# jolibrain/jolineedle

Measured on AMD Instinct MI355X. Metric: glimpse-patches/sec (448px, seq-len 20) REINFORCE step, higher is better.
Workload: dtype f32; 1 GPU; configs[2]/[3]: REINFORCE rollout, gpt-nano + yolox-nano encoder, 448px, seq-len 20, --enable-stop, 64 agents/GPU x 1 GPU, 4480x4480 synthetic images, forced non-STOP actions (S=T); global_batch=64, seq_len=20

## Files before the change

### include/jnroll.h

```cpp
#ifndef JNROLL_H
#define JNROLL_H

#include <stddef.h>
#include <stdint.h>

#ifdef __cplusplus
extern "C" {
#endif

#define JN_ABI_VERSION 2

enum {
  JN_OK = 0,
  JN_EINVAL = -1,
  JN_ENOMEM = -2,
  JN_EHIP = -3,
  JN_ENOTFOUND = -4,
  JN_ESTATE = -5
};

enum { JN_MODE_GREEDY = 0, JN_MODE_SAMPLE = 1, JN_MODE_FORCED = 2 };

enum { JN_NET_GPT_BACKBONE = 0, JN_NET_DETECTOR = 1 };

// ... 193 lines not shown

int jn_gpt_forward(jn_ctx* ctx, const float* patches_dev, const int64_t* actions_dev, const int64_t* classes_dev,
                   const int64_t* positions_dev, const float* prev_emb_dev, int B, int T, int Tp,
                   float* logits_dev, float* final_emb_dev, void* stream);
int jn_detect(jn_ctx* ctx, const float* patches_dev, int N, float* boxes_dev,
              int32_t* counts_dev, float* raw_dev, void* stream);
int jn_set_det_candidates(jn_ctx* ctx, int all);

int jn_detector_step(jn_ctx* ctx, const float* patches_dev, int N, const float* targets_dev, int nb,
                     float loss_scale, float* metrics_dev, void* stream);
#define JN_DETLOSS_MAX_BOXES 1024
int jn_set_det_loss_boxes(jn_ctx* ctx, int all);
int jn_detector_forward(jn_ctx* ctx, const float* patches_dev, int N, const float* targets_dev, int nb, int pass,
                        int n_pass, float* metrics_dev, float* boxes_dev, int32_t* counts_dev, float* fpn0_dev,
                        float* fpn1_dev, float* fpn2_dev, void* stream);
int jn_detector_backward(jn_ctx* ctx, int pass, const float* dloss_dev, float scale, void* stream);
int jn_detector_eval_loss(jn_ctx* ctx, const float* patches_dev, int N, const float* targets_dev, int nb,
                          float* metrics_dev, float* boxes_dev, int32_t* counts_dev, float* fpn0_dev, float* fpn1_dev,
                          float* fpn2_dev, void* stream);
int jn_optimizer_step_group(jn_ctx* ctx, int group, float lr, float weight_decay, float clip_value,
                            float grad_scale, void* stream);

int jn_rollout(jn_ctx* ctx, int mode, const int64_t* forced_actions_dev,
               const int64_t* start_positions_dev, uint64_t seed, int do_detection,
               int stop_early, const jn_rollout_out* out, void* stream);
int jn_set_rollout_positions(jn_ctx* ctx, int by_token);
int jn_teacher_actions(const int64_t* positions_dev, const uint8_t* visited_dev, const uint8_t* targets_dev, int B, int Gh,
                       int Gw, uint8_t* sets_dev, void* stream);
int jn_teacher_walks(const int64_t* bboxes_dev, const int64_t* start_positions_dev, int B, int nb, int Gh, int Gw, int P,
                     int T, int min_keypoints, int max_keypoints, int binomial_keypoints, uint64_t seed, int capacity,
                     int64_t* positions_dev, int64_t* current_actions_dev, int64_t* next_actions_dev, int64_t* labels_dev,
                     float* masks_dev, float* local_bboxes_dev, int32_t* n_steps_dev, uint8_t* targets_dev,
                     int64_t* cells_dev, float* bboxes_yolox_dev, int32_t* offsets_dev, void* stream);
int jn_set_rollout_teacher(jn_ctx* ctx, const uint8_t* targets_dev, uint8_t* sets_dev);
int jn_rollout_steps(jn_ctx* ctx, int* n_steps, void* stream);

int jn_last_timing(jn_ctx* ctx, int what, float* ms);
int jn_set_profiling(jn_ctx* ctx, int enabled);

#ifdef __cplusplus
}
#endif
#endif
```

### jolineedle_amd/_lib.py

```python
import ctypes as C
import os
from pathlib import Path

_LIB = None
LIB_PATH = Path(__file__).resolve().parent / "lib" / "libjnroll.so"

JN_MODE_GREEDY, JN_MODE_SAMPLE, JN_MODE_FORCED = 0, 1, 2
JN_NET_GPT_BACKBONE, JN_NET_DETECTOR = 0, 1


class LibraryNotBuilt(RuntimeError):
    pass


class JnError(RuntimeError):
    pass


class JnConfig(C.Structure):
    _fields_ = [("struct_size", C.c_int32), ("device", C.c_int32),
                ("n_layer", C.c_int32), ("n_head", C.c_int32), ("n_embd", C.c_int32),
                ("block_size", C.c_int32), ("n_actions", C.c_int32), ("patch_size", C.c_int32),
                ("use_pos_emb", C.c_int32), ("no_patch_emb", C.c_int32), ("concat_emb", C.c_int32),
                ("decoder_pos_encoding", C.c_int32), ("pos_emb_size", C.c_int32),
# ... 84 lines not shown
    "jn_pool_walk_detections": (C.c_int, [C.c_void_p] * 6 + [C.c_int] * 9 + [C.c_void_p] * 5),
    "jn_detection_cells": (C.c_int, [C.c_void_p, C.c_void_p] + [C.c_int] * 6 + [C.c_uint64, C.c_int] + [C.c_void_p] * 5),
    "jn_gather_patches_views": (C.c_int, [C.c_void_p, C.c_int, C.c_void_p, C.c_void_p, C.c_void_p, C.c_int, C.c_int, C.c_int,
                                          C.c_int, C.c_int, C.c_void_p]),
    "jn_backbone_forward": (C.c_int, [C.c_void_p, C.c_int, C.c_void_p, C.c_int, C.c_int, C.c_void_p, C.c_void_p,
                                      C.c_void_p, C.c_void_p]),
    "jn_read_tensor": (C.c_int, [C.c_void_p, C.c_char_p, C.c_void_p, C.c_size_t]),
    "jn_embed_patches": (C.c_int, [C.c_void_p, C.c_void_p, C.c_int, C.c_void_p, C.c_void_p]),
    "jn_reinforce_step": (C.c_int, [C.c_void_p, C.c_int, C.c_void_p, C.c_void_p, C.c_uint64, C.c_int,
                                    C.POINTER(JnTrainOpts), C.POINTER(JnRolloutOut), C.c_void_p, C.c_void_p]),
    "jn_supervised_step": (C.c_int, [C.c_void_p, C.c_void_p, C.c_void_p, C.c_void_p, C.c_void_p, C.c_void_p, C.c_void_p,
                                     C.c_int, C.c_int, C.c_float, C.c_void_p, C.c_void_p, C.c_void_p]),
    "jn_supervised_forward": (C.c_int, [C.c_void_p, C.c_void_p, C.c_void_p, C.c_void_p, C.c_void_p, C.c_int, C.c_int,
                                        C.c_void_p, C.c_void_p, C.c_void_p]),
    "jn_supervised_backward": (C.c_int, [C.c_void_p, C.c_void_p, C.c_void_p]),
    "jn_optimizer_step": (C.c_int, [C.c_void_p, C.c_float, C.c_float, C.c_float, C.c_float, C.c_void_p]),
    "jn_arena_info": (C.c_int, [C.c_void_p, C.POINTER(C.c_size_t), C.POINTER(C.c_size_t)]),
    "jn_set_grad_arena": (C.c_int, [C.c_void_p, C.c_void_p, C.c_size_t]),
    "jn_read_param": (C.c_int, [C.c_void_p, C.c_char_p, C.c_void_p, C.c_size_t]),
    "jn_zero_grad": (C.c_int, [C.c_void_p, C.c_void_p]),
    "jn_backbone_backward": (C.c_int, [C.c_void_p, C.c_int, C.c_void_p, C.c_int, C.c_void_p, C.c_void_p, C.c_void_p,
                                       C.c_void_p]),
    "jn_read_grad": (C.c_int, [C.c_void_p, C.c_char_p, C.c_void_p, C.c_size_t]),
    "jn_gpt_forward": (C.c_int, [C.c_void_p, C.c_void_p, C.c_void_p, C.c_void_p, C.c_void_p, C.c_void_p, C.c_int, C.c_int,
                                 C.c_int, C.c_void_p, C.c_void_p, C.c_void_p]),
    "jn_detect": (C.c_int, [C.c_void_p, C.c_void_p, C.c_int, C.c_void_p, C.c_void_p, C.c_void_p, C.c_void_p]),
    "jn_set_det_candidates": (C.c_int, [C.c_void_p, C.c_int]),
    "jn_set_det_loss_boxes": (C.c_int, [C.c_void_p, C.c_int]),
    "jn_rollout": (C.c_int, [C.c_void_p, C.c_int, C.c_void_p, C.c_void_p, C.c_uint64, C.c_int, C.c_int,
                             C.POINTER(JnRolloutOut), C.c_void_p]),
    "jn_set_rollout_positions": (C.c_int, [C.c_void_p, C.c_int]),
    "jn_teacher_actions": (C.c_int, [C.c_void_p, C.c_void_p, C.c_void_p, C.c_int, C.c_int, C.c_int, C.c_void_p, C.c_void_p]),
    "jn_teacher_walks": (C.c_int, [C.c_void_p, C.c_void_p] + [C.c_int] * 9 + [C.c_uint64, C.c_int] + [C.c_void_p] * 12),
    "jn_set_rollout_teacher":(C.c_int, [C.c_void_p, C.c_void_p, C.c_void_p]),
    "jn_rollout_steps": (C.c_int, [C.c_void_p, C.POINTER(C.c_int), C.c_void_p]),
    "jn_last_timing": (C.c_int, [C.c_void_p, C.c_int, C.POINTER(C.c_float)]),
    "jn_set_profiling": (C.c_int, [C.c_void_p, C.c_int]),
    "jn_detector_step": (C.c_int, [C.c_void_p, C.c_void_p, C.c_int, C.c_void_p, C.c_int, C.c_float, C.c_void_p, C.c_void_p]),
    "jn_detector_forward": (C.c_int, [C.c_void_p, C.c_void_p, C.c_int, C.c_void_p, C.c_int, C.c_int, C.c_int, C.c_void_p,
                                      C.c_void_p, C.c_void_p, C.c_void_p, C.c_void_p, C.c_void_p, C.c_void_p]),
    "jn_detector_backward": (C.c_int, [C.c_void_p, C.c_int, C.c_void_p, C.c_float, C.c_void_p]),
    "jn_optimizer_step_group": (C.c_int, [C.c_void_p, C.c_int, C.c_float, C.c_float, C.c_float, C.c_float, C.c_void_p]),
    "jn_reinforce_forward": (C.c_int, [C.c_void_p, C.c_int, C.c_void_p, C.c_void_p, C.c_uint64, C.c_int,
                                       C.POINTER(JnRolloutOut), C.c_void_p]),
    "jn_reinforce_backward": (C.c_int, [C.c_void_p, C.c_void_p, C.c_void_p, C.c_void_p]),
    "jn_arena_segment": (C.c_int, [C.c_void_p, C.c_char_p, C.POINTER(C.c_size_t), C.POINTER(C.c_size_t)]),
    "jn_export_arena": (C.c_int, [C.c_void_p, C.c_int, C.c_void_p, C.c_size_t, C.c_int, C.c_void_p]),
    "jn_import_arena": (C.c_int, [C.c_void_p, C.c_int, C.c_void_p, C.c_size_t, C.c_void_p]),
    "jn_set_dropout": (C.c_int, [C.c_void_p, C.c_float, C.c_uint64]),
    "jn_set_freeze": (C.c_int, [C.c_void_p, C.c_int]),
    "jn_optimizer_steps": (C.c_int, [C.c_void_p, C.c_int, C.POINTER(C.c_int), C.c_int]),
    "jn_supervised_metrics": (C.c_int, [C.c_void_p, C.c_void_p, C.c_void_p, C.c_void_p, C.c_int, C.c_int, C.c_int, C.c_float, C.c_int,
                                        C.c_void_p, C.c_void_p, C.c_void_p, C.c_void_p]),
    "jn_supervised_eval": (C.c_int, [C.c_void_p] * 7 + [C.c_int, C.c_int, C.c_float, C.c_int] + [C.c_void_p] * 5),
    "jn_detector_eval_loss": (C.c_int, [C.c_void_p, C.c_void_p, C.c_int, C.c_void_p, C.c_int] + [C.c_void_p] * 7),
}


def load_library(path=None):
    global _LIB
    if _LIB is not None and path is None:
        return _LIB
    p = Path(path or os.environ.get("JNROLL_LIB", LIB_PATH))
    if not p.exists():
        raise LibraryNotBuilt(
            f"{p} not found: the HIP extension is not built. Run `bash jolineedle_amd/csrc/build.sh` "
# ... 26 lines not shown
```

### jolineedle_amd/csrc/api_net.hip

```cpp
#include <algorithm>
#include <cstring>

#include "jn_internal.h"

using namespace jnr;

extern "C"
__global__ void bn_eval_table_kernel(const float* __restrict__ gamma, const float* __restrict__ beta,
                                     const float* __restrict__ rmean, const float* __restrict__ rvar, ChanTab t0,
                                     ChanTab t1, int C, float eps) {
  const int c = blockIdx.x * blockDim.x + threadIdx.x;
  if (c >= C) return;
  const float sc = gamma[c] / sqrtf(rvar[c] + eps);
  const float sh = beta[c] - rmean[c] * sc;
  t0.sc[c] = sc; t0.sh[c] = sh; t0.fl[c] = 1.0f;
  if (t1.sc) { t1.sc[c] = sc; t1.sh[c] = sh; t1.fl[c] = 1.0f; }
}

extern "C"
__global__ void fill_kernel(float* p, float v, long long n) {
  const long long i = (long long)blockIdx.x * blockDim.x + threadIdx.x;
  if (i < n) p[i] = v;
}

// ... 469 lines not shown
      } else {
        if (!st.red_by)
          launch_bn_bwd_reduce(gp_out, gld_out, ptr(op.out), net.act_dtype, ld(op.out), tab(op.out), save + 2 * cw.stat_off, cw.cout,
                               M, red, rep_stride, s, sb);
        launch_bn_bwd_consts(red, rep_stride, (double)M, cw.gamma_dev, cw.beta_dev, save + 2 * cw.stat_off, consts,
                             grad_of(ctx, cw.gamma_dev), grad_of(ctx, cw.beta_dev), cw.cout, s, sb, st.red_by & 1);
      }
      float* gw = grad_of(ctx, cw.w_dev);
      if (st.route == BR_PW_FUSED || st.route == BR_PW_FUSED_HALVES) {
        const int parts = st.route == BR_PW_FUSED ? 1 : 2, pc = cw.cout / parts;
        for (int part = 0; part < parts; ++part) {
          const int c0 = part * pc;
          ChanTab ot = tab(op.out);
          ot.sc += c0; ot.sh += c0; ot.fl += c0;
          PwBwdFusedArgs fa{};
          fa.g = gp_out + c0; fa.g_ld = gld_out; fa.z = (const float*)ptr(op.out) + c0; fa.z_ld = ld(op.out); fa.ot = ot;
          fa.save = save + 2 * (cw.stat_off + c0); fa.consts = consts + 3 * c0;
          fa.x = (const float*)ptr(op.in); fa.x_ld = ld(op.in); fa.it = tab(op.in); fa.w = cw.w_dev + (size_t)c0 * cw.cin;
          fa.gx = gptr(op.in); fa.gx_ld = ld(op.in); fa.accumulate = (op.acc_in || part > 0) ? 1 : 0;
          fa.gw = gw + (size_t)c0 * cw.cin; fa.wpart = ctx->wpart; fa.M = M; fa.cout = pc; fa.cin = cw.cin; fa.sb = sb;
          if (st.fold >= 0) {
            const View& sum = net.ops[st.fold].out;
            fa.gadd = gptr(sum); fa.gadd_ld = ld(sum); fa.accumulate = 0;
          }
          if (st.red_in >= 0 || st.red_in2 >= 0) fa.red_rep_stride = rep_stride;
          if (st.red_in >= 0) fa.red_in = sums(st.red_in, st.red_half);
          if (st.red_in2 >= 0) fa.red_in2 = sums(st.red_in2, st.red_half2);
          fa.red_split = st.red_split;
          if (st.red2) {
            const Op& co = net.ops[st.red_in];
            const ChanTab zt = tab(co.out);
            fa.red2_z = (const float*)ptr(co.out); fa.red2_ld = ld(co.out); fa.red2_sc = zt.sc; fa.red2_sh = zt.sh;
          }
          launch_pw_bwd_fused(fa, s);
        }
      } else if (st.route == BR_DW_FUSED) {
        DwBwdFusedArgs fa{};
        fa.g = gp_out; fa.g_ld = gld_out; fa.z = (const float*)ptr(op.out); fa.z_ld = ld(op.out); fa.ot = tab(op.out);
        fa.save = save + 2 * cw.stat_off; fa.consts = consts;
        fa.x = (const float*)ptr(op.in); fa.x_ld = ld(op.in); fa.it = tab(op.in); fa.w = cw.w_dev;
        fa.gin = gptr(op.in); fa.gin_ld = ld(op.in); fa.accumulate = op.acc_in ? 1 : 0; fa.gw = gw; fa.wpart = ctx->wpart;
        fa.C = cw.cout; fa.H = op.in.H; fa.W = op.in.W; fa.OH = op.out.H; fa.OW = op.out.W; fa.N = N; fa.stride = op.stride;
        fa.sb = sb;
        if (st.red_in >= 0) {
          fa.red_in = sums(st.red_in, st.red_half); fa.red_rep_stride = rep_stride;
          fa.accumulate = 0;
        }
        launch_dw_bwd_fused(fa, s);
      } else if (st.route == BR_STEM_FUSED) {
        StemArgs a{ss.src, ss.positions, ss.pos_stride, ss.sample_stride, ss.chan_stride, ss.row_stride, net.P, N, cw.cout,
                   cw.w_dev, nullptr, 0, JN_F32, nullptr, 0, nullptr, 0, 0, ss.src_u8};
        launch_stem_bwd_weight(a, gp_out, gld_out, gw, ctx->wpart, s, sb, (const float*)ptr(op.out), ld(op.out),
                               tab(op.out), save + 2 * cw.stat_off, consts);
      } else {
        launch_bn_bwd_gz(gp_out, gld_out, ptr(op.out), net.act_dtype, ld(op.out), tab(op.out), save + 2 * cw.stat_off, consts,
                         cw.cout, M, s, sb);
        if (st.route == BR_PW) {
          ConvArgs a{};
          a.in = gp_out; a.in_ld = gld_out; a.in_dtype = JN_F32; a.itab = ident; a.w = cw.w_dev; a.bias = nullptr;
          a.out = gptr(op.in); a.out_ld = ld(op.in); a.out_dtype = JN_F32; a.bf16_mfma = net.act_dtype == JN_BF16;
          a.N = N; a.H = op.out.H; a.W = op.out.W; a.OH = op.out.H; a.OW = op.out.W;
          a.cin = cw.cout; a.cout = cw.cin; a.stride = 1; a.act = ACT_NONE;
          a.accumulate = op.acc_in ? 1 : 0; a.w_transposed = 1; a.in_identity = 1;
          a.n_slots = nsl; a.in_slot_stride = sb.grad; a.out_slot_stride = sb.grad; a.tab_slot_stride = 0;
          hipStream_t ws = s;
          if (!no_aux && cw.cout >= 128 && cw.cin >= 128) {
// ... 199 lines not shown
```

### jolineedle_amd/csrc/api_ops.hip

```cpp
#include "jn_internal.h"

using namespace jnr;

template <typename T>
static int gather_patches(const char* who, bool indexed, const T* images_dev, const int64_t* image_index_dev,
                          const int64_t* positions_dev, float* out_dev, int N, int n_images, int C, int H, int W, int P, void* stream) {
  JN_CHECK(images_dev && (image_index_dev || !indexed) && positions_dev && out_dev, JN_EINVAL, "%s: null argument", who);
  JN_CHECK(N >= 0 && n_images >= 1 && C >= 1 && P >= 1 && H % P == 0 && W % P == 0, JN_EINVAL, "%s: bad shape", who);
  if (N == 0) return JN_OK;
  launch_gather(images_dev, positions_dev, out_dev, (long long)C * P * P, N, C, H, W, P, nullptr, 0, (hipStream_t)stream,
                image_index_dev);
  JN_HIP(hipGetLastError());
  return JN_OK;
}
extern "C" {

int jn_gather_patches(const float* images_dev, const int64_t* positions_dev, float* out_dev, int B, int C, int H, int W,
                      int P, void* stream) {
  return gather_patches("jn_gather_patches", false, images_dev, nullptr, positions_dev, out_dev, B, 1, C, H, W, P, stream);
}

int jn_gather_patches_u8(const uint8_t* images_dev, const int64_t* positions_dev, float* out_dev, int B, int C, int H,
                         int W, int P, void* stream) {
  return gather_patches("jn_gather_patches_u8", false, images_dev, nullptr, positions_dev, out_dev, B, 1, C, H, W, P, stream);
// ... 220 lines not shown

int jn_teacher_walks(const int64_t* bboxes_dev, const int64_t* start_positions_dev, int B, int nb, int Gh, int Gw, int P,
                     int T, int min_keypoints, int max_keypoints, int binomial_keypoints, uint64_t seed, int capacity,
                     int64_t* positions_dev, int64_t* current_actions_dev, int64_t* next_actions_dev, int64_t* labels_dev,
                     float* masks_dev, float* local_bboxes_dev, int32_t* n_steps_dev, uint8_t* targets_dev,
                     int64_t* cells_dev, float* bboxes_yolox_dev, int32_t* offsets_dev, void* stream) {
  JN_CHECK(B >= 0 && nb >= 0 && P >= 1 && capacity >= 0, JN_EINVAL, "jn_teacher_walks: B=%d nb=%d P=%d capacity=%d", B, nb, P,
           capacity);
  JN_CHECK(Gh >= 1 && Gw >= 1 && (long long)Gh * Gw <= JN_TWALK_MAX_CELLS, JN_EINVAL,
           "jn_teacher_walks: a grid of %d x %d cells, the kernel holds at most %d per image in LDS", Gh, Gw, JN_TWALK_MAX_CELLS);
  JN_CHECK(T >= 1 && T <= JN_TWALK_MAX_T, JN_EINVAL, "jn_teacher_walks: T=%d, the LDS ring holds 1..%d steps", T, JN_TWALK_MAX_T);
  JN_CHECK(min_keypoints >= 0 && max_keypoints >= min_keypoints && max_keypoints <= JN_TWALK_MAX_KEYPOINTS, JN_EINVAL,
           "jn_teacher_walks: min_keypoints=%d max_keypoints=%d, need 0 <= min <= max <= %d (the detour table)", min_keypoints,
           max_keypoints, JN_TWALK_MAX_KEYPOINTS);
  JN_CHECK((long long)B * Gh * Gw <= INT32_MAX, JN_EINVAL, "jn_teacher_walks: B * Gh * Gw beyond the int32 offsets");
  JN_CHECK(offsets_dev, JN_EINVAL, "jn_teacher_walks: null offsets");
  if (B == 0) {
    JN_HIP(hipMemsetAsync(offsets_dev, 0, sizeof(int32_t), (hipStream_t)stream));
    return JN_OK;
  }
  JN_CHECK(positions_dev && current_actions_dev && next_actions_dev && labels_dev && masks_dev && n_steps_dev && targets_dev,
           JN_EINVAL, "jn_teacher_walks: null output");
  JN_CHECK((bboxes_dev && local_bboxes_dev) || nb == 0, JN_EINVAL, "jn_teacher_walks: null boxes with nb=%d", nb);
  JN_CHECK((cells_dev && (bboxes_yolox_dev || nb == 0)) || capacity == 0, JN_EINVAL,
           "jn_teacher_walks: null detector rows with capacity=%d", capacity);
  TeacherWalkArgs a{bboxes_dev, start_positions_dev, B, nb, Gh, Gw, P, T, min_keypoints, max_keypoints,
                    binomial_keypoints != 0, seed, capacity, positions_dev, current_actions_dev, next_actions_dev, labels_dev,
                    masks_dev, local_bboxes_dev, n_steps_dev, targets_dev, cells_dev, bboxes_yolox_dev, offsets_dev};
  launch_teacher_walks(a, (hipStream_t)stream);
  JN_HIP(hipGetLastError());
  return JN_OK;
}

}
```

### jolineedle_amd/csrc/jn_kernels.h

```cpp
#pragma once
#include <hip/hip_runtime.h>

#include <cstdint>

#include "../../include/jnroll.h"

namespace jnr {

enum { ACT_NONE = 0, ACT_SILU = 1, ACT_RELU = 2, ACT_SIGMOID = 3 };
enum { JN_F32 = 0, JN_BF16 = 1 };

constexpr int JN_NREP = 32;
constexpr int JN_WPART_MAX = 16384;

struct ChanTab {
  float* sc; float* sh; float* fl;
  const int* dsrc;
  const float* dhw;
  const int* dgoff; const int* dboff;
  const float* dparams;
  const double* dstats;
  long long drep_stride;
  int dN;
  long long dmax;
// ... 129 lines not shown
                      int use_l1, float loss_scale, float* metrics, float* scale, hipStream_t s);
constexpr int DETLOSS_WIDE_MAX_A = 8400;
int launch_yolox_loss_wide(const float* raw, const float* labels, int N, int nb, const DetGeom& geo, float* d_raw, float* acc,
                           int use_l1, float loss_scale, float* metrics, float* scale, hipStream_t s);
int launch_head_pred_bwd(const float* d_raw, const float* scale, const void* reg, int reg_ld, ChanTab rt, const void* cls,
                         int cls_ld, ChanTab ct, int dtype, const float* wp, float* g_reg, float* g_cls, float* g_wp,
                         float* g_bp, int hid, int HW, int A, int a0, int N, hipStream_t s);

int launch_bn_bwd_reduce(const float* g, int g_ld, const void* z, int z_dtype, int z_ld, ChanTab t, const float* save,
                         int C, long long M, double* red_out, long long rep_stride, hipStream_t s,
                         const SlotBatch& sb = SlotBatch{});
int launch_bn_bwd_consts(const double* red, long long rep_stride, double count, const float* gamma, const float* beta,
                         const float* save, float* consts, float* g_gamma, float* g_beta, int C, hipStream_t s,
                         const SlotBatch& sb = SlotBatch{}, int raw_moment = 0);
int launch_bn_bwd_gz(float* g, int g_ld, const void* z, int z_dtype, int z_ld, ChanTab t, const float* save,
                     const float* consts, int C, long long M, hipStream_t s, const SlotBatch& sb = SlotBatch{});
int launch_pw_bwd_weight(const float* gz, int g_ld, const void* x, int x_dtype, int x_ld, ChanTab it, float* gw,
                         float* wpart, long long M, int N, int K, hipStream_t s, const SlotBatch& sb = SlotBatch{},
                         long long gz_slot_stride = -1);
int launch_wpart_reduce(float* gw, float* wpart, int n, hipStream_t s);
struct PwBwdFusedArgs {
  const float* g; int g_ld;
  const float* z; int z_ld; ChanTab ot;
  const float* save; const float* consts;
  const float* x; int x_ld; ChanTab it;
  const float* w;
  float* gx; int gx_ld; int accumulate;
  float* gw; float* wpart;
  long long M; int cout, cin;
  SlotBatch sb;
  double* red_in; long long red_rep_stride; double* red_in2; int red_split;
  const float* gadd; int gadd_ld;
  const float* red2_z; int red2_ld; const float* red2_sc; const float* red2_sh;
};
struct DwBwdFusedArgs {
  const float* g; int g_ld; const float* z; int z_ld; ChanTab ot; const float* save; const float* consts;
  const float* x; int x_ld; ChanTab it; const float* w;
  float* gin; int gin_ld; int accumulate; float* gw; float* wpart;
  int C, H, W, OH, OW, N, stride;
  SlotBatch sb;
  double* red_in; long long red_rep_stride;
};
bool dw_bwd_fused_supported(int C, int H, int W, int OH, int OW, int stride);
int launch_dw_bwd_fused(const DwBwdFusedArgs& a, hipStream_t s);
bool pw_bwd_fused_supported(int cout, int cin);
bool pw_bwd_fused_reduces_input(int cout, int cin);
int launch_pw_bwd_fused(const PwBwdFusedArgs& a, hipStream_t s);
int launch_dw_bwd_data(const float* gz, int g_ld, const float* w, float* gin, int gin_ld, int C, int H, int W, int OH,
                       int OW, int N, int stride, int accumulate, hipStream_t s, const SlotBatch& sb = SlotBatch{});
int launch_dw_bwd_weight(const float* gz, int g_ld, const void* x, int x_dtype, int x_ld, ChanTab it, float* gw,
                         float* wpart, int C, int H, int W, int OH, int OW, int N, int stride, hipStream_t s,
                         const SlotBatch& sb = SlotBatch{});
int launch_stem_bwd_weight(const StemArgs& a, const float* gz, int g_ld, float* gw, float* wpart, hipStream_t s,
                           const SlotBatch& sb = SlotBatch{}, const float* z = nullptr, int z_ld = 0,
                           ChanTab ot = ChanTab{nullptr, nullptr, nullptr}, const float* save = nullptr,
                           const float* consts = nullptr);
int launch_spp_bwd(const void* cat, int dtype, float* gcat, int ld, int h, int H, int W, int N, ChanTab it,
                   hipStream_t s, const SlotBatch& sb = SlotBatch{});
int launch_upsample_bwd(const float* gdst, int dst_ld, float* gsrc, int src_ld, int C, int H, int W, int N,
                        int accumulate, hipStream_t s, const SlotBatch& sb = SlotBatch{});
int launch_grad_copy(const float* src, int src_ld, float* dst, int dst_ld, int C, long long M, int accumulate,
                     hipStream_t s, const SlotBatch& sb = SlotBatch{});
int launch_nchw_to_nhwc_grad(const float* in, float* out, int out_ld, int C, int HW, int N, int accumulate,
                             hipStream_t s);

#ifndef JN_DW_S2_PAD
#define JN_DW_S2_PAD 4
#endif
constexpr int AUG_NPARAM = 20;
int launch_augment(const float* in, float* out, const float* params, const float* noise, unsigned long long seed, int N, int P,
                   hipStream_t s);
int launch_gather(const float* images, const int64_t* positions, float* out, long long out_sample_stride,
                  int B, int C, int H, int W, int P, const int* skip_flag, int skip_when, hipStream_t s,
                  const int64_t* image_index = nullptr);
int launch_gather(const uint8_t* images, const int64_t* positions, float* out, long long out_sample_stride,
                  int B, int C, int H, int W, int P, const int* skip_flag, int skip_when, hipStream_t s,
                  const int64_t* image_index = nullptr);
// ... 156 lines not shown
```

### jolineedle_amd/csrc/kernels_bwd.hip

```cpp
#include <hip/hip_runtime.h>

#include <algorithm>
#include <cstdlib>
#include <type_traits>

#include "jn_kernels.h"
#include "jn_reduce.h"
#include "jn_types.h"

namespace jnr {

__device__ __forceinline__ float sigmoidf_(float v) { return __builtin_amdgcn_rcpf(1.0f + __expf(-v)); }
__device__ __forceinline__ float silu_(float v) { return v * sigmoidf_(v); }
__device__ __forceinline__ float dsilu_(float y) {
  const float s = sigmoidf_(y);
  return s * (1.0f + y * (1.0f - s));
}
__device__ __forceinline__ f32x4 tf4_(f32x4 z, f32x4 sc, f32x4 sh, f32x4 fl) {
  f32x4 r;
  r.x = fl.x != 0.0f ? silu_(fmaf(z.x, sc.x, sh.x)) : z.x;
  r.y = fl.y != 0.0f ? silu_(fmaf(z.y, sc.y, sh.y)) : z.y;
  r.z = fl.z != 0.0f ? silu_(fmaf(z.z, sc.z, sh.z)) : z.z;
  r.w = fl.w != 0.0f ? silu_(fmaf(z.w, sc.w, sh.w)) : z.w;
  return r;
// ... 691 lines not shown
              float* tp = &Ts[(16 * a + 4 * gq + r) * K + 16 * b + lm];
              *tp = (wv == 0 ? 0.0f : *tp) + dw[a][b][r];
            }
      }
    }
  }
  __syncthreads();
  float* dst = rep ? gw + ((blockIdx.x + 5 * blockIdx.y) % JN_NREP) * JN_WPART_MAX : gw;
  for (int i = tid; i < N * K; i += 256) atomicAdd(&dst[i], Ts[i]);
}

template <int CTN, int CTK, bool RED, bool RED2 = false>
static void launch_pw_bwd_fused_r(const PwBwdFusedArgs& a, hipStream_t s) {
  constexpr int N = 16 * CTN, K = 16 * CTK;
  size_t smem = ((size_t)64 * (N + 4) + 64 * (K + 4) + (size_t)K * (N + 4) + 7 * N + 3 * K + (RED ? (RED2 ? 10 : 8) * K : 0)) * sizeof(float);
  if (smem < (size_t)N * K * sizeof(float)) smem = (size_t)N * K * sizeof(float);
  if (smem > 64 * 1024) {
    static bool raised = false;
    if (!raised) {
      (void)hipFuncSetAttribute(reinterpret_cast<const void*>(&pw_bwd_fused_kernel<CTN, CTK, RED, RED2>),
                                hipFuncAttributeMaxDynamicSharedMemorySize, (int)smem);
      raised = true;
    }
  }
  const long long n_tiles = (a.M + 63) / 64;
  static int places = 0;
  if (!places) {
    int per_cu = 0;
    if (hipOccupancyMaxActiveBlocksPerMultiprocessor(&per_cu, reinterpret_cast<const void*>(&pw_bwd_fused_kernel<CTN, CTK, RED, RED2>), 256, smem) != hipSuccess || per_cu < 1) per_cu = 2;
    places = per_cu * 256;
  }
  const int rounds = std::max(1, (1024 + places / 2) / places);
  long long bx = (long long)rounds * places / a.sb.n;
  if (bx < 1) bx = 1;
  if (bx > n_tiles) bx = n_tiles;
  const int rep = (a.wpart && N * K <= JN_WPART_MAX) ? 1 : 0;
  hipLaunchKernelGGL((pw_bwd_fused_kernel<CTN, CTK, RED, RED2>), dim3((unsigned)bx, a.sb.n), dim3(256), smem, s, a.g, a.g_ld, a.z,
                     a.z_ld, a.ot, a.save, a.consts, a.x, a.x_ld, a.it, a.w, a.gx, a.gx_ld, a.accumulate,
                     rep ? a.wpart : a.gw, rep, a.M, a.sb, a.red_in, a.red_rep_stride, a.gadd, a.gadd_ld, a.red_in2,
                     a.red_split > 0 ? a.red_split : K, a.red2_z, a.red2_ld, a.red2_sc, a.red2_sh);
  if (rep) launch_wpart_reduce(a.gw, a.wpart, N * K, s);
}

template <int CTN, int CTK>
static void launch_pw_bwd_fused_t(const PwBwdFusedArgs& a, hipStream_t s) {
  if constexpr (CTK <= 4) {
    if (a.red2_z) { launch_pw_bwd_fused_r<CTN, CTK, true, true>(a, s); return; }
    if (a.red_in || a.red_in2) { launch_pw_bwd_fused_r<CTN, CTK, true>(a, s); return; }
  }
  launch_pw_bwd_fused_r<CTN, CTK, false>(a, s);
}

bool pw_bwd_fused_reduces_input(int cout, int cin) { return pw_bwd_fused_supported(cout, cin) && cin <= 64; }

bool pw_bwd_fused_supported(int cout, int cin) {
  if (cout % 16 || cin % 16) return false;
  const int tn = cout / 16, tk = cin / 16;
  auto pow2 = [](int v) { return v == 1 || v == 2 || v == 4 || v == 8; };
  return pow2(tn) && pow2(tk);
}

int launch_pw_bwd_fused(const PwBwdFusedArgs& a, hipStream_t s) {
  const int tn = a.cout / 16, tk = a.cin / 16;
#define JN_PF(A, B) if (tn == A && tk == B) { launch_pw_bwd_fused_t<A, B>(a, s); return 0; }
  JN_PF(1, 1) JN_PF(1, 2) JN_PF(1, 4) JN_PF(1, 8) JN_PF(2, 1) JN_PF(2, 2) JN_PF(2, 4) JN_PF(2, 8)
  JN_PF(4, 1) JN_PF(4, 2) JN_PF(4, 4) JN_PF(4, 8) JN_PF(8, 1) JN_PF(8, 2) JN_PF(8, 4) JN_PF(8, 8)
#undef JN_PF
  return -1;
}

template <int S>
__global__ __launch_bounds__(256) void dw_bwd_data_kernel(const float* __restrict__ gz, int g_ld,
                                                          const float* __restrict__ w, float* __restrict__ gin,
                                                          int gin_ld, int C, int H, int W, int OH, int OW, int N,
                                                          int accumulate, long long g_slot) {
  gz += blockIdx.y * g_slot; gin += blockIdx.y * g_slot;
  const int C4 = C >> 2;
  const long long total = (long long)N * H * W * C4;
  const long long idx = (long long)blockIdx.x * 256 + threadIdx.x;
  if (idx >= total) return;
  const int c = (int)(idx % C4) * 4;
  const int ix = (int)((idx / C4) % W);
  const int iy = (int)((idx / ((long long)C4 * W)) % H);
  const long long n = idx / ((long long)C4 * W * H);
  f32x4 acc = {0.f, 0.f, 0.f, 0.f};
#pragma unroll
  for (int ky = 0; ky < 3; ++ky) {
    const int ty = iy + 1 - ky;
    if (ty < 0 || (S == 2 && (ty & 1))) continue;
    const int oy = ty / S;
    if (oy >= OH) continue;
#pragma unroll
    for (int kx = 0; kx < 3; ++kx) {
      const int tx = ix + 1 - kx;
      if (tx < 0 || (S == 2 && (tx & 1))) continue;
      const int ox = tx / S;
// ... 803 lines not shown
```

### jolineedle_amd/csrc/kernels_pwxs.hip

```cpp
#include <hip/hip_runtime.h>

#include <algorithm>
#include <cstdlib>

#include "jn_kernels.h"
#include "jn_reduce.h"
#include "jn_tab.h"
#include "jn_types.h"

namespace jnr {

struct UpsDst { float* out; int ld; int W; int HW; };
template <bool UPS>
__device__ __forceinline__ void ups_store(const UpsDst& u, long long m, int n, const f32x4& v) {
  if constexpr (UPS) {
    const long long img = m / u.HW;
    const int rem = (int)(m - img * u.HW), y = rem / u.W, x = rem - y * u.W;
    float* d = u.out + ((img * 2 * (u.HW / u.W) + 2 * y) * (2LL * u.W) + 2 * x) * u.ld + n;
    *reinterpret_cast<f32x4*>(d) = v;
    *reinterpret_cast<f32x4*>(d + u.ld) = v;
    d += 2LL * u.W * u.ld;
    *reinterpret_cast<f32x4*>(d) = v;
    *reinterpret_cast<f32x4*>(d + u.ld) = v;
  }
// ... 496 lines not shown
#endif
  JN_X3(64, 1, 2, 2) JN_X3(64, 2, 2, 2) JN_X3(128, 1, 2, 4) JN_X3(128, 2, 2, 4) JN_X3(128, 4, 2, 2)
  JN_X3(256, 2, 2, 2) JN_X3(256, 4, 4, 2) JN_X3(512, 4, 2, 2)
#ifdef JN_X3_ALL_SHAPES
  JN_X3(64, 1, 4, 2) JN_X3(64, 2, 4, 2) JN_X3(128, 1, 4, 4) JN_X3(128, 2, 4, 4) JN_X3(128, 4, 4, 2)
  JN_X3(256, 2, 4, 2) JN_X3(256, 4, 2, 2)
#endif
#undef JN_X3
  return -1;
}

__global__ __launch_bounds__(256) void w_split3_t_kernel(const float* __restrict__ w, bf16_t* __restrict__ w3t, int cout, int cin) {
  const int i = blockIdx.x * 256 + threadIdx.x;
  const int groups = cout / 8;
  if (i >= cin * groups) return;
  const int n = i % cin, gq = i / cin;
  const int NJ = cout / 32, j = gq >> 2, g = gq & 3;
  bf16x8 h, m, l;
#pragma unroll
  for (int e = 0; e < 8; ++e) {
    const float v = w[(long long)(8 * gq + e) * cin + n];
    const bf16_t vh = (bf16_t)v;
    const float r1 = v - (float)vh;
    const bf16_t vm = (bf16_t)r1;
    const float r2 = r1 - (float)vm;
    h[e] = vh; m[e] = vm; l[e] = (bf16_t)r2;
  }
  bf16_t* o = w3t + ((long long)((n >> 4) * NJ + j) * 3 * 64 + g * 16 + (n & 15)) * 8;
  *reinterpret_cast<bf16x8*>(o) = h;
  *reinterpret_cast<bf16x8*>(o + 512) = m;
  *reinterpret_cast<bf16x8*>(o + 1024) = l;
}

bool pw_x3_bwd_data_supported(int cout, int cin) {
  return (cout == 256 && (cin == 128 || cin == 256 || cin == 512)) || (cout == 128 && cin == 256);
}

int launch_pw_x3_bwd_data(const ConvArgs& a, const float* w, void* w3t, hipStream_t s) {
  const int K = a.cin, N = a.cout;
  if (!pw_x3_bwd_data_supported(K, N) || a.accumulate || a.in_dtype != JN_F32 || a.out_dtype != JN_F32 || a.bias ||
      a.act != ACT_NONE || a.in_ld % 4 != 0 || a.out_ld % 4 != 0 || a.stats)
    return -1;
  hipLaunchKernelGGL(w_split3_t_kernel, dim3((unsigned)((N * (K / 8) + 255) / 256)), dim3(256), 0, s, w, (bf16_t*)w3t, K, N);
  const long long M = (long long)a.N * a.H * a.W;
  ConvArgs b = a;
  b.w_x3 = w3t; b.up_out = nullptr;
  if (K == 256 && N == 128) { launch_pw_x3_t<256, 2, 2, 2, 3, float, false, true>(b, M, 2, s); return 0; }
  if (K == 128 && N == 256) { launch_pw_x3_t<128, 4, 2, 4, 3, float, false, true>(b, M, 2, s); return 0; }
  for (int n0 = 0; n0 < N; n0 += 256) {
    b.w_x3 = (const bf16_t*)w3t + (long long)n0 * K * 3;
    b.out = (float*)a.out + n0;
    launch_pw_x3_t<256, 4, 2, 2, 3, float, false, true>(b, M, 2, s);
  }
  return 0;
}

}
```

Before: 13270 glimpse-patches/s.

## Add specialized MFMA fused pointwise backward kernel for 128-input-channel convs

```diff
diff --git a/include/jnroll.h b/include/jnroll.h
--- a/include/jnroll.h
+++ b/include/jnroll.h
@@ -249,6 +249,9 @@
                      int64_t* positions_dev, int64_t* current_actions_dev, int64_t* next_actions_dev, int64_t* labels_dev,
                      float* masks_dev, float* local_bboxes_dev, int32_t* n_steps_dev, uint8_t* targets_dev,
                      int64_t* cells_dev, float* bboxes_yolox_dev, int32_t* offsets_dev, void* stream);
+int jn_pw_bwd_fused(const float* g_dev, const float* z_dev, const float* x_dev, const float* tab_dev, const float* save_dev,
+                    const float* consts_dev, const float* w_dev, const float* gadd_dev, int accumulate, float* gx_dev,
+                    float* gw_dev, int S, long long M, int cout, int cin, int route, int max_wg, void* stream);
 int jn_set_rollout_teacher(jn_ctx* ctx, const uint8_t* targets_dev, uint8_t* sets_dev);
 int jn_rollout_steps(jn_ctx* ctx, int* n_steps, void* stream);
 
diff --git a/jolineedle_amd/_lib.py b/jolineedle_amd/_lib.py
--- a/jolineedle_amd/_lib.py
+++ b/jolineedle_amd/_lib.py
@@ -140,6 +140,7 @@
     "jn_set_rollout_positions": (C.c_int, [C.c_void_p, C.c_int]),
     "jn_teacher_actions": (C.c_int, [C.c_void_p, C.c_void_p, C.c_void_p, C.c_int, C.c_int, C.c_int, C.c_void_p, C.c_void_p]),
     "jn_teacher_walks": (C.c_int, [C.c_void_p, C.c_void_p] + [C.c_int] * 9 + [C.c_uint64, C.c_int] + [C.c_void_p] * 12),
+    "jn_pw_bwd_fused": (C.c_int, [C.c_void_p] * 8 + [C.c_int] + [C.c_void_p] * 2 + [C.c_int, C.c_longlong] + [C.c_int] * 4 + [C.c_void_p]),
     "jn_set_rollout_teacher":(C.c_int, [C.c_void_p, C.c_void_p, C.c_void_p]),
     "jn_rollout_steps": (C.c_int, [C.c_void_p, C.POINTER(C.c_int), C.c_void_p]),
     "jn_last_timing": (C.c_int, [C.c_void_p, C.c_int, C.POINTER(C.c_float)]),
diff --git a/jolineedle_amd/csrc/api_net.hip b/jolineedle_amd/csrc/api_net.hip
--- a/jolineedle_amd/csrc/api_net.hip
+++ b/jolineedle_amd/csrc/api_net.hip
@@ -525,6 +525,8 @@
             const ChanTab zt = tab(co.out);
             fa.red2_z = (const float*)ptr(co.out); fa.red2_ld = ld(co.out); fa.red2_sc = zt.sc; fa.red2_sh = zt.sh;
           }
+          if (net.act_dtype == JN_F32 && ctx->params_x3t && cw.cin == 128 && (pc == 128 || pc == 64) && (fa.w - ctx->params) % 8 == 0)
+            fa.w_frag = reinterpret_cast<float*>(ctx->params_x3t + 3 * (fa.w - ctx->params));
           launch_pw_bwd_fused(fa, s);
         }
       } else if (st.route == BR_DW_FUSED) {
diff --git a/jolineedle_amd/csrc/api_ops.hip b/jolineedle_amd/csrc/api_ops.hip
--- a/jolineedle_amd/csrc/api_ops.hip
+++ b/jolineedle_amd/csrc/api_ops.hip
@@ -276,4 +276,53 @@
   return JN_OK;
 }
 
-}
+int jn_pw_bwd_fused(const float* g_dev, const float* z_dev, const float* x_dev, const float* tab_dev, const float* save_dev,
+                    const float* consts_dev, const float* w_dev, const float* gadd_dev, int accumulate, float* gx_dev,
+                    float* gw_dev, int S, long long M, int cout, int cin, int route, int max_wg, void* stream) {
+  JN_CHECK(g_dev && z_dev && x_dev && tab_dev && save_dev && consts_dev && w_dev && gx_dev && gw_dev, JN_EINVAL,
+           "jn_pw_bwd_fused: null argument");
+  JN_CHECK(S >= 1 && M >= 1 && M <= (1LL << 40), JN_EINVAL, "jn_pw_bwd_fused: S=%d M=%lld", S, M);
+  JN_CHECK(cout >= 16 && cin >= 16 && pw_bwd_fused_supported(cout, cin), JN_EINVAL, "jn_pw_bwd_fused: %d -> %d channels: no fused kernel",
+           cin, cout);
+  JN_CHECK((route == 0 || route == 1) && max_wg >= 0, JN_EINVAL, "jn_pw_bwd_fused: route=%d max_wg=%d", route, max_wg);
+  hipStream_t s = (hipStream_t)stream;
+  const long long C = cout + cin;
+  const size_t zn = (size_t)M * cout, xn = (size_t)M * cin, act = zn + xn, grad = zn + 2 * xn;
+  float* ws = nullptr;
+  JN_HIP(hipMalloc((void**)&ws, ((size_t)S * (act + grad) + (size_t)2 * cout * cin) * sizeof(float)));
+  float *za = ws, *xa = za + zn, *ga = ws + (size_t)S * act, *gxa = ga + zn, *gadda = gxa + xn, *w_frag = ws + (size_t)S * (act + grad);
+  auto lay = [&](float* dst, size_t dst_slot, const float* src, size_t n, bool back) {
+    return back ? hipMemcpy2DAsync(const_cast<float*>(src), n * sizeof(float), dst, dst_slot * sizeof(float), n * sizeof(float), S, hipMemcpyDeviceToDevice, s)
+                : hipMemcpy2DAsync(dst, dst_slot * sizeof(float), src, n * sizeof(float), n * sizeof(float), S, hipMemcpyDeviceToDevice, s);
+  };
+  hipError_t e = lay(za, act, z_dev, zn, false);
+  if (e == hipSuccess) e = lay(xa, act, x_dev, xn, false);
+  if (e == hipSuccess) e = lay(ga, grad, g_dev, zn, false);
+  if (e == hipSuccess && accumulate) e = lay(gxa, grad, gx_dev, xn, false);
+  if (e == hipSuccess && gadd_dev) e = lay(gadda, grad, gadd_dev, xn, false);
+  int rc = -1;
+  if (e == hipSuccess) {
+    float* tab = const_cast<float*>(tab_dev);
+    PwBwdFusedArgs a{};
+    a.g = ga; a.g_ld = cout; a.z = za; a.z_ld = cout;
+    a.ot.sc = tab; a.ot.sh = tab + C; a.ot.fl = tab + 2 * C;
+    a.save = save_dev; a.consts = consts_dev;
+    a.x = xa; a.x_ld = cin;
+    a.it.sc = tab + cout; a.it.sh = tab + C + cout; a.it.fl = tab + 2 * C + cout;
+    a.w = w_dev; a.gx = gxa; a.gx_ld = cin; a.accumulate = accumulate ? 1 : 0; a.gw = gw_dev;
+    a.M = M; a.cout = cout; a.cin = cin;
+    a.sb.n = S; a.sb.act = (long long)act; a.sb.grad = (long long)grad; a.sb.tab = 3 * C; a.sb.save = 2LL * cout; a.sb.consts = 3LL * cout;
+    if (gadd_dev) { a.gadd = gadda; a.gadd_ld = cin; }
+    a.w_frag = w_frag; a.route = route; a.max_wg = max_wg;
+    rc = launch_pw_bwd_fused(a, s);
+    e = hipGetLastError();
+    if (e == hipSuccess) e = lay(gxa, grad, gx_dev, xn, true);
+  }
+  if (e == hipSuccess) e = hipStreamSynchronize(s);
+  (void)hipFree(ws);
+  JN_HIP(e);
+  JN_CHECK(rc == 0, JN_EINVAL, "jn_pw_bwd_fused: %d -> %d channels: no fused kernel", cin, cout);
+  return JN_OK;
+}
+
+}
diff --git a/jolineedle_amd/csrc/jn_kernels.h b/jolineedle_amd/csrc/jn_kernels.h
--- a/jolineedle_amd/csrc/jn_kernels.h
+++ b/jolineedle_amd/csrc/jn_kernels.h
@@ -185,6 +185,9 @@
   double* red_in; long long red_rep_stride; double* red_in2; int red_split;
   const float* gadd; int gadd_ld;
   const float* red2_z; int red2_ld; const float* red2_sc; const float* red2_sh;
+  float* w_frag;
+  int route;
+  int max_wg;
 };
 struct DwBwdFusedArgs {
   const float* g; int g_ld; const float* z; int z_ld; ChanTab ot; const float* save; const float* consts;
@@ -196,6 +199,7 @@
 };
 bool dw_bwd_fused_supported(int C, int H, int W, int OH, int OW, int stride);
 int launch_dw_bwd_fused(const DwBwdFusedArgs& a, hipStream_t s);
+int launch_w_split3_t(const float* w, void* w3t, int cout, int cin, hipStream_t s);
 bool pw_bwd_fused_supported(int cout, int cin);
 bool pw_bwd_fused_reduces_input(int cout, int cin);
 int launch_pw_bwd_fused(const PwBwdFusedArgs& a, hipStream_t s);
diff --git a/jolineedle_amd/csrc/kernels_bwd.hip b/jolineedle_amd/csrc/kernels_bwd.hip
--- a/jolineedle_amd/csrc/kernels_bwd.hip
+++ b/jolineedle_amd/csrc/kernels_bwd.hip
@@ -747,6 +747,7 @@
   }
   const int rounds = std::max(1, (1024 + places / 2) / places);
   long long bx = (long long)rounds * places / a.sb.n;
+  if (a.max_wg > 0 && bx > a.max_wg / a.sb.n) bx = a.max_wg / a.sb.n;
   if (bx < 1) bx = 1;
   if (bx > n_tiles) bx = n_tiles;
   const int rep = (a.wpart && N * K <= JN_WPART_MAX) ? 1 : 0;
@@ -766,6 +767,312 @@
   launch_pw_bwd_fused_r<CTN, CTK, false>(a, s);
 }
 
+
+using gfloat_p = const __attribute__((address_space(1))) float*;
+__device__ __forceinline__ gfloat_p pin_uniform(const float* p) {
+  asm volatile("" : "+s"(p));
+  return (gfloat_p)p;
+}
+__device__ __forceinline__ f32x4 ldg4(gfloat_p base, unsigned off) {
+  return *(const __attribute__((address_space(1))) f32x4*)(base + off);
+}
+
+__global__ __launch_bounds__(256) void w_frag_t_kernel(const float* __restrict__ w, float* __restrict__ wf, int N, int K) {
+  const int i = blockIdx.x * 256 + threadIdx.x;
+  if (i >= N * K / 4) return;
+  const int lane = i & 63, lm = lane & 15, gq = lane >> 4, NS = N / 16, s = (i >> 6) % NS, b = (i >> 6) / NS;
+  f32x4 v;
+#pragma unroll
+  for (int j = 0; j < 4; ++j) v[j] = w[(long long)(16 * s + 4 * gq + j) * K + 16 * b + lm];
+  *reinterpret_cast<f32x4*>(wf + 4LL * i) = v;
+}
+
+template <int CTN, int D, bool X3>
+__global__ __launch_bounds__(256, 2) void pw_bwd_fused128_kernel(
+    const float* __restrict__ g, int g_ld, const float* __restrict__ z, int z_ld, ChanTab ot,
+    const float* __restrict__ save, const float* __restrict__ consts, const float* __restrict__ x, int x_ld,
+    ChanTab it, const float* __restrict__ wf, float* __restrict__ gx, int gx_ld, int accumulate,
+    float* __restrict__ gw, int rep, long long M, SlotBatch sb, const float* __restrict__ gadd, int gadd_ld) {
+  constexpr int N = 16 * CTN, K = 128, NS = N / 16;
+  constexpr int LDG = N + 4, LDA = K + 4;
+  constexpr int NG = 32 * (N / 4) / 256, NA = 32 * (K / 4) / 256;
+  constexpr int NJ = N / 32, LDK = N + 16;
+  static_assert(NG >= 1 && D >= 1 && D < (X3 ? 2 * NJ : NS), "pw_bwd_fused128 tile mapping");
+  constexpr int TILE = 32 * LDG + 32 * LDA, NBUF = X3 ? 1 : 2;
+  __shared__ __attribute__((aligned(16))) float sm[NBUF * TILE + 7 * N + 3 * K + (X3 ? 3 * 32 * LDK / 2 : 0)];
+  float* Gs = sm;
+  float* As = Gs + 32 * LDG;
+  float* const Cs = sm + NBUF * TILE;
+  bf16_t* const Gp = reinterpret_cast<bf16_t*>(Cs + 7 * N + 3 * K);
+  const int tid = threadIdx.x, lane = tid & 63, wave = tid >> 6;
+  const int lm = lane & 15, gq = lane >> 4;
+  const int nq = tid % (N / 4), kq = tid % (K / 4);
+  const long long tiles_per_slot = (M + 31) / 32, n_tiles = tiles_per_slot * sb.n;
+  const long long t_begin = n_tiles * blockIdx.x / gridDim.x, t_end = n_tiles * (blockIdx.x + 1) / gridDim.x;
+  if (t_begin >= t_end) return;
+
+  constexpr int DW_AN = CTN / 2, DW_BN = 4;
+  const int dw_a0 = (wave & 1) * DW_AN, dw_b0 = (wave >> 1) * DW_BN;
+  f32x4 dw[DW_AN][DW_BN];
+#pragma unroll
+  for (int a = 0; a < DW_AN; ++a)
+#pragma unroll
+    for (int b = 0; b < DW_BN; ++b) dw[a][b] = f32x4{0.f, 0.f, 0.f, 0.f};
+
+  f32x4 rg[NG], rz[NG], rx[NA];
+  long long f_slot = 0, f_m0 = 0;
+  auto fetch = [&](bool next) {
+    if (next) {
+      f_m0 += 32;
+      if (f_m0 >= M) { f_m0 = 0; ++f_slot; }
+    }
+    const gfloat_p gs = pin_uniform(g + f_slot * sb.grad + f_m0 * g_ld), zs = pin_uniform(z + f_slot * sb.act + f_m0 * z_ld),
+                   xs = pin_uniform(x + f_slot * sb.act + f_m0 * x_ld);
+    const int last = (int)(M - f_m0 < 32 ? M - f_m0 : 32) - 1;
+#pragma unroll
+    for (int j = 0; j < NG; ++j) {
+      const int r = std::min((tid + 256 * j) / (N / 4), last);
+      rg[j] = ldg4(gs, r * g_ld + 4 * nq);
+      rz[j] = ldg4(zs, r * z_ld + 4 * nq);
+    }
+#pragma unroll
+    for (int j = 0; j < NA; ++j) {
+      const int r = std::min((tid + 256 * j) / (K / 4), last);
+      rx[j] = ldg4(xs, r * x_ld + 4 * kq);
+    }
+  };
+  f32x4 eo[2][2];
+  auto fetch_store_operand = [&](long long slot, long long m0) {
+    const gfloat_p src = pin_uniform(gadd ? gadd + slot * sb.grad + m0 * gadd_ld : gx + slot * sb.grad + m0 * gx_ld);
+    const int src_ld = gadd ? gadd_ld : gx_ld;
+    const int last = (int)(M - m0 < 32 ? M - m0 : 32) - 1;
+#pragma unroll
+    for (int c = 0; c < 2; ++c)
+#pragma unroll
+      for (int p = 0; p < 2; ++p)
+        eo[c][p] = ldg4(src, std::min(16 * p + lm, last) * src_ld + 16 * (2 * wave + c) + 4 * gq);
+  };
+  auto load_consts = [&](long long sl) {
+    const gfloat_p o_sc = pin_uniform(ot.sc + sl * sb.tab), o_sh = pin_uniform(ot.sh + sl * sb.tab), sv = pin_uniform(save + sl * sb.save),
+                   cn = pin_uniform(consts + sl * sb.consts);
+    for (int c = tid; c < N; c += 256) {
+      Cs[c] = o_sc[c]; Cs[N + c] = o_sh[c]; Cs[2 * N + c] = sv[2 * c]; Cs[3 * N + c] = sv[2 * c + 1];
+      Cs[4 * N + c] = cn[3 * c]; Cs[5 * N + c] = cn[3 * c + 1]; Cs[6 * N + c] = cn[3 * c + 2];
+    }
+    const gfloat_p i_sc = pin_uniform(it.sc + sl * sb.tab), i_sh = pin_uniform(it.sh + sl * sb.tab), i_fl = pin_uniform(it.fl + sl * sb.tab);
+    for (int c = tid; c < K; c += 256) { Cs[7 * N + c] = i_sc[c]; Cs[7 * N + K + c] = i_sh[c]; Cs[7 * N + 2 * K + c] = i_fl[c]; }
+  };
+  auto stage = [&](long long m0) {
+#pragma unroll
+    for (int j = 0; j < NG; ++j) {
+      const int r = (tid + 256 * j) / (N / 4);
+      f32x4 v = {0.f, 0.f, 0.f, 0.f};
+      if (m0 + r < M) {
+        const f32x4 o_sc = *reinterpret_cast<const f32x4*>(Cs + 4 * nq), o_sh = *reinterpret_cast<const f32x4*>(Cs + N + 4 * nq),
+                    o_mean = *reinterpret_cast<const f32x4*>(Cs + 2 * N + 4 * nq), o_istd = *reinterpret_cast<const f32x4*>(Cs + 3 * N + 4 * nq),
+                    o_c1 = *reinterpret_cast<const f32x4*>(Cs + 4 * N + 4 * nq), o_c2 = *reinterpret_cast<const f32x4*>(Cs + 5 * N + 4 * nq),
+                    o_k = *reinterpret_cast<const f32x4*>(Cs + 6 * N + 4 * nq);
+#pragma unroll
+        for (int q = 0; q < 4; ++q) {
+          const float zh = (rz[j][q] - o_mean[q]) * o_istd[q];
+          const float gy = rg[j][q] * dsilu_(fmaf(rz[j][q], o_sc[q], o_sh[q]));
+          v[q] = o_k[q] * (gy - o_c1[q] - zh * o_c2[q]);
+        }
+      }
+      *reinterpret_cast<f32x4*>(Gs + r * LDG + 4 * nq) = v;
+      if constexpr (X3) {
+        const bf16x4 vh = __builtin_convertvector(v, bf16x4);
+        const f32x4 r1 = v - __builtin_convertvector(vh, f32x4);
+        const bf16x4 vm = __builtin_convertvector(r1, bf16x4);
+        const f32x4 r2 = r1 - __builtin_convertvector(vm, f32x4);
+        bf16_t* dst = Gp + r * LDK + 4 * nq;
+        *reinterpret_cast<bf16x4*>(dst) = vh;
+        *reinterpret_cast<bf16x4*>(dst + 32 * LDK) = vm;
+        *reinterpret_cast<bf16x4*>(dst + 2 * 32 * LDK) = __builtin_convertvector(r2, bf16x4);
+      }
+    }
+#pragma unroll
+    for (int j = 0; j < NA; ++j) {
+      const int r = (tid + 256 * j) / (K / 4);
+      f32x4 v = {0.f, 0.f, 0.f, 0.f};
+      if (m0 + r < M)
+        v = tf4_(rx[j], *reinterpret_cast<const f32x4*>(Cs + 7 * N + 4 * kq), *reinterpret_cast<const f32x4*>(Cs + 7 * N + K + 4 * kq),
+                 *reinterpret_cast<const f32x4*>(Cs + 7 * N + 2 * K + 4 * kq));
+      *reinterpret_cast<f32x4*>(As + r * LDA + 4 * kq) = v;
+    }
+  };
+
+  gfloat_p wbase = pin_uniform(wf);
+  const unsigned woff = (2 * wave * NS * 64 + lane) * 4;
+  auto wfrag = [&](int c, int s) -> f32x4 { return ldg4(wbase, woff + (c * NS + s) * 256); };
+  auto wfrag3 = [&](int c, int j, int t) -> bf16x8 {
+    return __builtin_bit_cast(bf16x8, ldg4(wbase, (((2 * wave + c) * NJ + j) * 3 + t) * 256 + lane * 4));
+  };
+
+  long long cur_slot = -1;
+  f_slot = t_begin / tiles_per_slot;
+  f_m0 = (t_begin - f_slot * tiles_per_slot) * 32;
+  fetch(false);
+#pragma unroll 1
+  for (long long tile = t_begin; tile < t_end; ++tile) {
+    const long long slot = f_slot, m0 = f_m0;
+    f32x4 wa[X3 ? 1 : NS][2];
+    bf16x8 wx[X3 ? 2 * NJ : 1][3];
+    wbase = pin_uniform(wf);
+#pragma unroll
+    for (int s = 0; s < D; ++s) {
+      if constexpr (X3) {
+#pragma unroll
+        for (int t = 0; t < 3; ++t) wx[s][t] = wfrag3(s & 1, s >> 1, t);
+      } else {
+#pragma unroll
+        for (int c = 0; c < 2; ++c) wa[s][c] = wfrag(c, s);
+      }
+    }
+    if constexpr (NBUF == 1) __syncthreads();
+    if (slot != cur_slot) {
+      load_consts(slot);
+      cur_slot = slot;
+      __syncthreads();
+    }
+    if constexpr (NBUF == 2) {
+      Gs = sm + ((tile - t_begin) & 1) * TILE;
+      As = Gs + 32 * LDG;
+    }
+    stage(m0);
+    __syncthreads();
+    f32x4 acc[2][2];
+#pragma unroll
+    for (int c = 0; c < 2; ++c)
+#pragma unroll
+      for (int p = 0; p < 2; ++p) acc[c][p] = f32x4{0.f, 0.f, 0.f, 0.f};
+    auto late_loads = [&]() {
+      if (gadd || accumulate) fetch_store_operand(slot, m0);
+      fetch(tile + 1 < t_end);
+    };
+    if constexpr (X3) {
+      const bf16_t* xrow = Gp + lm * LDK + 8 * gq;
+#pragma unroll
+      for (int u = 0; u < 2 * NJ; ++u) {
+        const int j = u >> 1, c = u & 1;
+        if (u + D < 2 * NJ) {
+#pragma unroll
+          for (int t = 0; t < 3; ++t) wx[u + D][t] = wfrag3((u + D) & 1, (u + D) >> 1, t);
+        }
+        if (u + D == 2 * NJ - 1) late_loads();
+        __builtin_amdgcn_sched_barrier(0);
+        constexpr int TW[6] = {2, 0, 1, 1, 0, 0}, TX[6] = {0, 2, 1, 0, 1, 0};
+#pragma unroll
+        for (int p = 0; p < 2; ++p) {
+          bf16x8 xa[3];
+#pragma unroll
+          for (int t = 0; t < 3; ++t) xa[t] = *reinterpret_cast<const bf16x8*>(xrow + t * 32 * LDK + p * 16 * LDK + 32 * j);
+#pragma unroll
+          for (int e = 0; e < 6; ++e) acc[c][p] = __builtin_amdgcn_mfma_f32_16x16x32_bf16(wx[u][TW[e]], xa[TX[e]], acc[c][p], 0, 0, 0);
+        }
+      }
+    } else {
+      const float* grow = Gs + lm * LDG + 4 * gq;
+#pragma unroll
+      for (int s = 0; s < NS; ++s) {
+        if (s + D < NS) {
+#pragma unroll
+          for (int c = 0; c < 2; ++c) wa[s + D][c] = wfrag(c, s + D);
+        }
+        if (s + D == NS - 1) late_loads();
+        __builtin_amdgcn_sched_barrier(0);
+        f32x4 gb[2];
+#pragma unroll
+        for (int p = 0; p < 2; ++p) gb[p] = *reinterpret_cast<const f32x4*>(grow + p * 16 * LDG + 16 * s);
+#pragma unroll
+        for (int c = 0; c < 2; ++c)
+#pragma unroll
+          for (int p = 0; p < 2; ++p)
+#pragma unroll
+            for (int j = 0; j < 4; ++j) acc[c][p] = __builtin_amdgcn_mfma_f32_16x16x4f32(wa[s][c][j], gb[p][j], acc[c][p], 0, 0, 0);
+      }
+    }
+    {
+      float* gxs = gx + slot * sb.grad + m0 * gx_ld;
+#pragma unroll
+      for (int c = 0; c < 2; ++c)
+#pragma unroll
+        for (int p = 0; p < 2; ++p)
+          if (m0 + 16 * p + lm < M) {
+            float* op = gxs + (unsigned)((16 * p + lm) * gx_ld + 16 * (2 * wave + c) + 4 * gq);
+            f32x4 v = acc[c][p];
+            if (gadd || accumulate) v += eo[c][p];
+            if (gadd && accumulate) v += *reinterpret_cast<const f32x4*>(op);
+            *reinterpret_cast<f32x4*>(op) = v;
+          }
+    }
+    {
+      const int prow = 4 * gq;
+      bf16x8 bh[DW_BN], bl[DW_BN];
+#pragma unroll
+      for (int b = 0; b < DW_BN; ++b)
+#pragma unroll
+        for (int e = 0; e < 8; ++e) {
+          const float v = As[(prow + (e & 3) + 16 * (e >> 2)) * LDA + 16 * (dw_b0 + b) + lm];
+          const bf16_t h = (bf16_t)v;
+          bh[b][e] = h; bl[b][e] = (bf16_t)(v - (float)h);
+        }
+#pragma unroll
+      for (int a = 0; a < DW_AN; ++a) {
+        bf16x8 ah, al;
+#pragma unroll
+        for (int e = 0; e < 8; ++e) {
+          const float v = Gs[(prow + (e & 3) + 16 * (e >> 2)) * LDG + 16 * (dw_a0 + a) + lm];
+          const bf16_t h = (bf16_t)v;
+          ah[e] = h; al[e] = (bf16_t)(v - (float)h);
+        }
+#pragma unroll
+        for (int b = 0; b < DW_BN; ++b) {
+          f32x4 d = dw[a][b];
+          d = __builtin_amdgcn_mfma_f32_16x16x32_bf16(ah, bh[b], d, 0, 0, 0);
+          d = __builtin_amdgcn_mfma_f32_16x16x32_bf16(ah, bl[b], d, 0, 0, 0);
+          d = __builtin_amdgcn_mfma_f32_16x16x32_bf16(al, bh[b], d, 0, 0, 0);
+          dw[a][b] = d;
+        }
+      }
+    }
+  }
+  float* dst = rep ? gw + (blockIdx.x % JN_NREP) * JN_WPART_MAX : gw;
+#pragma unroll
+  for (int a = 0; a < DW_AN; ++a)
+#pragma unroll
+    for (int b = 0; b < DW_BN; ++b)
+#pragma unroll
+      for (int r = 0; r < 4; ++r) atomicAdd(&dst[(16 * (dw_a0 + a) + 4 * gq + r) * K + 16 * (dw_b0 + b) + lm], dw[a][b][r]);
+}
+
+template <int CTN, int D, bool X3>
+static void launch_pw_bwd_fused128(const PwBwdFusedArgs& a, hipStream_t s) {
+  constexpr int N = 16 * CTN, K = 128;
+  if (X3) launch_w_split3_t(a.w, a.w_frag, N, K, s);
+  else hipLaunchKernelGGL(w_frag_t_kernel, dim3(N * K / 4 / 256), dim3(256), 0, s, a.w, a.w_frag, N, K);
+  static int places = 0;
+  if (!places) {
+    int per_cu = 0;
+    if (hipOccupancyMaxActiveBlocksPerMultiprocessor(&per_cu, reinterpret_cast<const void*>(&pw_bwd_fused128_kernel<CTN, D, X3>), 256, 0) != hipSuccess || per_cu < 1) per_cu = 2;
+    places = per_cu * 256;
+  }
+  const long long n_tiles = (a.M + 31) / 32 * a.sb.n;
+  long long bx = std::min<long long>(places, n_tiles);
+  if (a.max_wg > 0) bx = std::min<long long>(bx, a.max_wg);
+  const int rep = (a.wpart && N * K <= JN_WPART_MAX) ? 1 : 0;
+  hipLaunchKernelGGL((pw_bwd_fused128_kernel<CTN, D, X3>), dim3((unsigned)bx), dim3(256), 0, s, a.g, a.g_ld, a.z, a.z_ld, a.ot, a.save,
+                     a.consts, a.x, a.x_ld, a.it, a.w_frag, a.gx, a.gx_ld, a.accumulate, rep ? a.wpart : a.gw, rep, a.M, a.sb,
+                     a.gadd, a.gadd_ld);
+  if (rep) launch_wpart_reduce(a.gw, a.wpart, N * K, s);
+}
+
+static bool pw_bwd_fused128_takes(const PwBwdFusedArgs& a) {
+  return a.w_frag && a.route != 1 && a.cin == 128 && (a.cout == 128 || a.cout == 64) && !a.red_in && !a.red_in2 && !a.red2_z &&
+         a.g_ld % 4 == 0 && a.z_ld % 4 == 0 && a.x_ld % 4 == 0 && a.gx_ld % 4 == 0 && (!a.gadd || a.gadd_ld % 4 == 0) &&
+         reinterpret_cast<uintptr_t>(a.w_frag) % 16 == 0;
+}
+
 bool pw_bwd_fused_reduces_input(int cout, int cin) { return pw_bwd_fused_supported(cout, cin) && cin <= 64; }
 
 bool pw_bwd_fused_supported(int cout, int cin) {
@@ -777,6 +1084,10 @@
 
 int launch_pw_bwd_fused(const PwBwdFusedArgs& a, hipStream_t s) {
   const int tn = a.cout / 16, tk = a.cin / 16;
+  if (pw_bwd_fused128_takes(a)) {
+    if (tn == 8) launch_pw_bwd_fused128<8, 2, true>(a, s); else launch_pw_bwd_fused128<4, 2, false>(a, s);
+    return 0;
+  }
 #define JN_PF(A, B) if (tn == A && tk == B) { launch_pw_bwd_fused_t<A, B>(a, s); return 0; }
   JN_PF(1, 1) JN_PF(1, 2) JN_PF(1, 4) JN_PF(1, 8) JN_PF(2, 1) JN_PF(2, 2) JN_PF(2, 4) JN_PF(2, 8)
   JN_PF(4, 1) JN_PF(4, 2) JN_PF(4, 4) JN_PF(4, 8) JN_PF(8, 1) JN_PF(8, 2) JN_PF(8, 4) JN_PF(8, 8)
diff --git a/jolineedle_amd/csrc/kernels_pwxs.hip b/jolineedle_amd/csrc/kernels_pwxs.hip
--- a/jolineedle_amd/csrc/kernels_pwxs.hip
+++ b/jolineedle_amd/csrc/kernels_pwxs.hip
@@ -552,6 +552,11 @@
   *reinterpret_cast<bf16x8*>(o + 1024) = l;
 }
 
+int launch_w_split3_t(const float* w, void* w3t, int cout, int cin, hipStream_t s) {
+  hipLaunchKernelGGL(w_split3_t_kernel, dim3((unsigned)((cin * (cout / 8) + 255) / 256)), dim3(256), 0, s, w, (bf16_t*)w3t, cout, cin);
+  return 0;
+}
+
 bool pw_x3_bwd_data_supported(int cout, int cin) {
   return (cout == 256 && (cin == 128 || cin == 256 || cin == 512)) || (cout == 128 && cin == 256);
 }
@@ -561,7 +566,7 @@
   if (!pw_x3_bwd_data_supported(K, N) || a.accumulate || a.in_dtype != JN_F32 || a.out_dtype != JN_F32 || a.bias ||
       a.act != ACT_NONE || a.in_ld % 4 != 0 || a.out_ld % 4 != 0 || a.stats)
     return -1;
-  hipLaunchKernelGGL(w_split3_t_kernel, dim3((unsigned)((N * (K / 8) + 255) / 256)), dim3(256), 0, s, w, (bf16_t*)w3t, K, N);
+  launch_w_split3_t(w, w3t, K, N, s);
   const long long M = (long long)a.N * a.H * a.W;
   ConvArgs b = a;
   b.w_x3 = w3t; b.up_out = nullptr;
```

New measurement: 13510 glimpse-patches/s (median of 6 runs). +1.8%, better.
